# PaddlePaddle/Paddle3D

Measured on AMD Instinct MI355X. Metric: scenes/sec CenterPoint-Pillars nuScenes 300k-pt sweeps, higher is better.
Workload: dtype f32

## Files before the change

include/paddle3d_amd.h:

```cpp
#ifndef PADDLE3D_AMD_H
#define PADDLE3D_AMD_H

#include <stddef.h>
#include <stdint.h>

#ifdef __cplusplus
extern "C" {
#endif

#define PD3_OK 0
#define PD3_EINVAL (-1)
#define PD3_EWORKSPACE (-2)
#define PD3_EUNSUPPORTED (-3)

int pd3_version(void);
const char *pd3_target_arch(void);

int pd3_selfcheck_lds_atomic_order(const uint32_t *addr, uint32_t *old, int blocks, int waves_per_block, int rounds,
                                   int table, void *stream);

size_t pd3_hard_voxelize_workspace(int batch, int64_t max_points, int num_point_dim,
                                   const float *voxel_size, const float *point_cloud_range,
                                   int max_num_points_in_voxel, int max_voxels);
int pd3_hard_voxelize(const float *points, const int32_t *num_points, int batch, int64_t max_points,
                      int num_point_dim, const float *voxel_size, const float *point_cloud_range,
                      int max_num_points_in_voxel, int max_voxels, float *voxels, int32_t *coords,
                      int32_t *num_points_per_voxel, int32_t *num_voxels, int32_t *coors_batched,
                      void *workspace, size_t workspace_bytes, void *stream);
int pd3_hard_voxelize_path(const float *points, const int32_t *num_points, int batch, int64_t max_points,
                           int num_point_dim, const float *voxel_size, const float *point_cloud_range,
                           int max_num_points_in_voxel, int max_voxels, float *voxels, int32_t *coords,
                           int32_t *num_points_per_voxel, int32_t *num_voxels, int32_t *coors_batched,
                           void *workspace, size_t workspace_bytes, void *stream, int path);

int64_t pd3_hard_voxelize_index_list_entries(int batch, int64_t max_points);
int pd3_hard_voxelize_index(const float *points, const int32_t *num_points, int batch, int64_t max_points,
                            int num_point_dim, const float *voxel_size, const float *point_cloud_range,
                            int max_num_points_in_voxel, int max_voxels, int32_t *vox_span, int32_t *point_list,
                            int32_t *coords, int32_t *num_points_per_voxel, int32_t *num_voxels,
                            int32_t *coors_batched, void *workspace, size_t workspace_bytes, void *stream);

int pd3_hard_voxelize_f64(const double *points, const int32_t *num_points, int batch, int64_t max_points,
                          int num_point_dim, const float *voxel_size, const float *point_cloud_range,
                          int max_num_points_in_voxel, int max_voxels, double *voxels, int32_t *coords,
                          int32_t *num_points_per_voxel, int32_t *num_voxels, int32_t *coors_batched,
                          void *workspace, size_t workspace_bytes, void *stream);

int pd3_dynamic_voxelize(const float *points, int64_t num_points, int num_point_dim, const float *voxel_size,
                         const float *point_cloud_range, int32_t *coors, void *stream);

size_t pd3_pointpillars_scatter_workspace(int batch, int ny, int nx);
int pd3_pointpillars_scatter(const float *voxel_features, const int32_t *coords,
                             int64_t num_pillars, int channels, int batch, int ny, int nx,
                             float *canvas, void *workspace, size_t workspace_bytes, void *stream);

int pd3_pointpillars_inverse_map(const int32_t *coords, int64_t num_pillars, int batch, int ny, int nx,
                                 int32_t *inv, void *stream);
int pd3_scatter_conv3x3_bias_relu(const float *voxel_features, const int32_t *inv, const float *w_packed,
                                  const float *bias, int batch, int cin, int cout, int ny, int nx, int stride,
                                  int relu, float *out, int out_w, void *stream);

size_t pd3_pillar_conv_rulebook_workspace(int batch, int ny, int nx, int stride);
int pd3_pillar_conv_rulebook(const int32_t *inverse_map, int batch, int ny, int nx, int stride, int32_t *nbr,
                             int32_t *out_cell, int32_t *cell_row, int32_t *n_out, int capacity, int32_t *order,
                             void *workspace, size_t workspace_bytes, void *stream);
int pd3_rows_to_dense_fill(const float *rows, const int32_t *cell_row, const float *fill, int batch, int channels, int h,
                           int w, float *out, void *stream);

int pd3_pillar_feature_net(const float *voxels, const int32_t *num_points, const int32_t *coors,
                           int64_t num_pillars, int max_points, int num_point_dim,
                           int voxel_center_dims, float vx, float vy, float vz, float x_offset,
                           float y_offset, float z_offset, const float *w1, const float *scale1,
                           const float *shift1, int c1, const float *w2, const float *scale2,
                           const float *shift2, int c2, float *out, void *stream);

int pd3_pillar_feature_net_path(const float *voxels, const int32_t *num_points, const int32_t *coors,
                                int64_t num_pillars, int max_points, int num_point_dim,
                                int voxel_center_dims, float vx, float vy, float vz, float x_offset,
                                float y_offset, float z_offset, const float *w1, const float *scale1,
                                const float *shift1, int c1, const float *w2, const float *scale2,
                                const float *shift2, int c2, float *out, int path, void *stream);

int pd3_pillar_feature_net_indexed(const float *points, int64_t points_per_frame, const int32_t *vox_span,
                                   const int32_t *point_list, int64_t list_stride, const int32_t *coors,
                                   int64_t num_pillars, int pillars_per_frame, int max_points, int num_point_dim,
                                   int voxel_center_dims, float vx, float vy, float vz, float x_offset,
                                   float y_offset, float z_offset, const float *w1, const float *scale1,
                                   const float *shift1, int c1, const float *w2, const float *scale2,
                                   const float *shift2, int c2, float *out, void *stream);

int pd3_voxel_mean(const float *voxels, const int32_t *num_points, int64_t num_voxels,
                   int max_points, int num_point_dim, float *out, void *stream);

size_t pd3_nms_workspace(int num_boxes);
int pd3_nms_bev(const float *boxes, int num_boxes, float nms_overlap_thresh, int32_t *keep,
                int32_t *num_to_keep, void *workspace, size_t workspace_bytes, void *stream);
int pd3_nms_normal(const float *boxes, int num_boxes, float nms_overlap_thresh, int32_t *keep,
                   int32_t *num_to_keep, void *workspace, size_t workspace_bytes, void *stream);
int pd3_boxes_iou_bev(const float *boxes_a, int num_a, const float *boxes_b, int num_b,
                      float *ans_iou, void *stream);
int pd3_boxes_overlap_bev(const float *boxes_a, int num_a, const float *boxes_b, int num_b,
                          float *ans_overlap, void *stream);
int pd3_libm_eval(int op, const float *x, const float *y, float *out, int64_t n, void *stream);

size_t pd3_centerpoint_postprocess_workspace(int batch, int num_tasks, int feat_h, int feat_w,
                                             int nms_pre_max_size, int nms_post_max_size);
int pd3_centerpoint_postprocess(const float *const *hm, const float *const *reg,
                                const float *const *height, const float *const *dim,
                                const float *const *vel, const float *const *rot, int batch,
                                int num_tasks, const int *hm_channels, int feat_h, int feat_w,
                                const float *voxel_size, const float *point_cloud_range,
                                const float *post_center_range, const int *label_offsets,
                                int down_ratio, float score_threshold, float nms_iou_threshold,
                                int nms_pre_max_size, int nms_post_max_size, int with_velocity,
                                float *out_bboxes, float *out_scores, int64_t *out_labels,
                                int32_t *out_count, void *workspace, size_t workspace_bytes,
                                void *stream);

int pd3_centerpoint_postprocess_strided(const float *const *hm, const float *const *reg,
                                const float *const *height, const float *const *dim,
                                const float *const *vel, const float *const *rot, int64_t head_batch_stride, int batch,
                                int num_tasks, const int *hm_channels, int feat_h, int feat_w,
                                const float *voxel_size, const float *point_cloud_range,
                                const float *post_center_range, const int *label_offsets,
                                int down_ratio, float score_threshold, float nms_iou_threshold,
                                int nms_pre_max_size, int nms_post_max_size, int with_velocity,
                                float *out_bboxes, float *out_scores, int64_t *out_labels,
                                int32_t *out_count, void *workspace, size_t workspace_bytes,
                                void *stream, int selection);
int pd3_centerpoint_postprocess_records(const float *const *hm, const float *const *reg,
                                        const float *const *height, const float *const *dim,
                                        const float *const *vel, const float *const *rot,
                                        int64_t head_batch_stride, int batch, int num_tasks,
                                        const int *hm_channels, int feat_h, int feat_w, const float *voxel_size,
                                        const float *point_cloud_range, const float *post_center_range,
                                        const int *label_offsets, int down_ratio, float score_threshold,
                                        float nms_iou_threshold, int nms_pre_max_size, int nms_post_max_size,
                                        int with_velocity, float *out_bboxes, float *out_scores,
                                        int64_t *out_labels, int32_t *out_count, float *out_records,
                                        int max_per_img, void *workspace, size_t workspace_bytes, void *stream);

size_t pd3_bevdet_postprocess_workspace(int batch, int num_tasks, const int *task_classes, int feat_h, int feat_w,
                                        int max_num);
int pd3_bevdet_postprocess(const float *const *heatmap, const float *const *reg, const float *const *height,
                           const float *const *dim, const float *const *rot, const float *const *vel, int batch,
                           int num_tasks, const int *task_classes, int feat_h, int feat_w, const int *nms_type,
                           const float *nms_thr, const double *min_radius, const float *rescale_factors,
                           int max_num, int pre_max_size, int post_max_size, float score_threshold, int norm_bbox,
                           const float *post_center_range, const float *post_center_limit_range,
                           const float *pc_range, const float *voxel_size, float out_size_factor,
// ... 325 lines not shown
```

paddle3d_amd/_lib.py:

```python
from __future__ import annotations

import ctypes as C
import os
from functools import lru_cache

_HERE = os.path.dirname(os.path.abspath(__file__))
LIB_PATH = os.path.join(_HERE, "lib", "libpaddle3d_amd.so")

c_f32p = C.c_void_p
c_i32p = C.c_void_p

_SIGNATURES = {
    "pd3_version": (C.c_int, []),
    "pd3_target_arch": (C.c_char_p, []),
    "pd3_hard_voxelize_workspace": (C.c_size_t, [C.c_int, C.c_int64, C.c_int, C.c_void_p, C.c_void_p,
                                                 C.c_int, C.c_int]),
    "pd3_hard_voxelize": (C.c_int, [C.c_void_p, C.c_void_p, C.c_int, C.c_int64, C.c_int, C.c_void_p,
                                    C.c_void_p, C.c_int, C.c_int, C.c_void_p, C.c_void_p, C.c_void_p,
                                    C.c_void_p, C.c_void_p, C.c_void_p, C.c_size_t, C.c_void_p]),
    "pd3_hard_voxelize_f64": (C.c_int, [C.c_void_p, C.c_void_p, C.c_int, C.c_int64, C.c_int, C.c_void_p,
                                    C.c_void_p, C.c_int, C.c_int, C.c_void_p, C.c_void_p, C.c_void_p,
                                    C.c_void_p, C.c_void_p, C.c_void_p, C.c_size_t, C.c_void_p]),
    "pd3_hard_voxelize_path": (C.c_int, [C.c_void_p, C.c_void_p, C.c_int, C.c_int64, C.c_int, C.c_void_p,
                                         C.c_void_p, C.c_int, C.c_int, C.c_void_p, C.c_void_p, C.c_void_p,
# ... 199 lines not shown

_SIGNATURES_ROI = {
    "pd3_voxel_pool": (C.c_int, [C.c_void_p] * 8 + [C.c_int] * 7 + [C.c_float] + [C.c_int] * 5 + [C.c_void_p] * 2),
    "pd3_roi_grid_points": (C.c_int, [C.c_void_p, C.c_int64, C.c_int, C.c_int] + [C.c_void_p] * 3 + [C.c_int] +
                            [C.c_void_p] * 3),
    "pd3_rcnn_decode_boxes": (C.c_int, [C.c_void_p, C.c_void_p, C.c_int64, C.c_void_p, C.c_void_p]),
    "pd3_class_agnostic_nms_workspace": (C.c_size_t, [C.c_int, C.c_int64, C.c_int]),
    "pd3_class_agnostic_nms": (C.c_int, [C.c_void_p, C.c_void_p, C.c_int, C.c_int64, C.c_int, C.c_int, C.c_float,
                                         C.c_void_p, C.c_int, C.c_float, C.c_int] + [C.c_void_p] * 5 +
                               [C.c_size_t, C.c_void_p]),
}

SYMBOLS_ROI = tuple(_SIGNATURES_ROI)

_SIGNATURES_HEAD = {
    "pd3_grouped_conv3x3_small_counts_slice": (C.c_int, [C.c_void_p, C.c_void_p, C.c_void_p, C.c_int, C.c_int, C.c_int,
                                                         C.c_int, C.c_void_p, C.c_int, C.c_int, C.c_void_p, C.c_int,
                                                         C.c_int, C.c_void_p]),
}

SYMBOLS_HEAD = tuple(_SIGNATURES_HEAD)

_SIGNATURES_PVRCNN = {
    "pd3_stack_sa_pool": (C.c_int, [C.c_void_p] * 11 + [C.c_int] * 5 + [C.c_float, C.c_int] + [C.c_void_p] * 2),
    "pd3_bev_interpolate": (C.c_int, [C.c_void_p, C.c_void_p, C.c_int64] + [C.c_int] * 4 + [C.c_float] * 5 +
                            [C.c_void_p] * 2),
}

SYMBOLS_PVRCNN = tuple(_SIGNATURES_PVRCNN)

_CADDN_GRID = [C.c_int] * 3 + [C.c_void_p] * 2 + [C.c_int, C.c_double, C.c_double]
_CADDN_IN = [C.c_void_p] * 5 + [C.c_int] * 5 + _CADDN_GRID
_SIGNATURES_CADDN = {
    "pd3_frustum_grid": (C.c_int, [C.c_void_p] * 3 + [C.c_int] + _CADDN_GRID + [C.c_int] + [C.c_void_p] * 2),
    "pd3_frustum_to_voxel_workspace": (C.c_size_t, [C.c_int] * 5),
    "pd3_frustum_to_voxel": (C.c_int, _CADDN_IN + [C.c_void_p, C.c_void_p, C.c_size_t, C.c_void_p]),
    "pd3_frustum_to_bev_workspace": (C.c_size_t, [C.c_int] * 7),
    "pd3_frustum_to_bev": (C.c_int, _CADDN_IN + [C.c_void_p] * 3 + [C.c_int, C.c_void_p, C.c_void_p, C.c_size_t,
                                                                    C.c_void_p]),
}

SYMBOLS_CADDN = tuple(_SIGNATURES_CADDN)

_SIGNATURES_BEVFORMER = {
    "pd3_bevformer_point_sampling": (C.c_int, [C.c_void_p] * 3 + [C.c_int] * 6 + [C.c_void_p] * 5),
    "pd3_bevformer_sca": (C.c_int, [C.c_void_p] * 7 + [C.c_int] * 9 + [C.c_void_p] * 2),
    "pd3_bevformer_tsa": (C.c_int, [C.c_void_p] * 6 + [C.c_int] * 7 + [C.c_void_p] * 2),
}

SYMBOLS_BEVFORMER = tuple(_SIGNATURES_BEVFORMER)

_SIGNATURES_BEVFORMER_DEC = {
    "pd3_mha_forward": (C.c_int, [C.c_void_p] * 3 + [C.c_int] * 5 + [C.c_float] + [C.c_void_p] * 2),
    "pd3_bevformer_dec_ca": (C.c_int, [C.c_void_p] * 6 + [C.c_int] * 8 + [C.c_void_p] * 2),
    "pd3_nms_free_decode": (C.c_int, [C.c_void_p] * 3 + [C.c_int] * 5 + [C.c_double, C.c_int] + [C.c_void_p] * 5),
}

SYMBOLS_BEVFORMER_DEC = tuple(_SIGNATURES_BEVFORMER_DEC)

_SIGNATURES_PETR = {
    "pd3_mha_stream_forward": (C.c_int, [C.c_void_p] * 4 + [C.c_int] * 5 + [C.c_float] + [C.c_void_p] * 2),
    "pd3_petr_coords3d": (C.c_int, [C.c_void_p] + [C.c_int] * 6 + [C.c_double, C.c_void_p, C.c_int] + [C.c_void_p] * 4),
}

SYMBOLS_PETR = tuple(_SIGNATURES_PETR)

_SIGNATURES_SQSEG = {
    "pd3_sac_isk_forward": (C.c_int, [C.c_void_p] * 8 + [C.c_int] * 4 + [C.c_void_p] * 2),
    "pd3_range_project": (C.c_int, [C.c_void_p, C.c_int64, C.c_void_p] + [C.c_int] * 3 + [C.c_double] * 2 +
                          [C.c_void_p] * 8 + [C.c_size_t, C.c_void_p]),
}

SYMBOLS_SQSEG = tuple(_SIGNATURES_SQSEG)

_A3D_CFG = [C.c_int] * 2 + [C.c_float] * 4 + [C.c_void_p] * 5 + [C.c_size_t, C.c_void_p]
_SIGNATURES_ANCHOR3D = {
    "pd3_anchor3d_head_workspace": (C.c_size_t, [C.c_int] * 7),
    "pd3_anchor3d_head_forward": (C.c_int, [C.c_void_p] * 8 + [C.c_int] * 7 + _A3D_CFG),
    "pd3_anchor3d_get_bboxes": (C.c_int, [C.c_void_p] * 4 + [C.c_int] * 6 + _A3D_CFG),
}

SYMBOLS_ANCHOR3D = tuple(_SIGNATURES_ANCHOR3D)


class Paddle3DAmdError(RuntimeError):
    pass


@lru_cache(maxsize=None)
def lib() -> C.CDLL:
    if not os.path.exists(LIB_PATH):
        raise Paddle3DAmdError(
            f"{LIB_PATH} not found: build it with `python -m paddle3d_amd.build` "
            "(there is no CPU / PyTorch fallback for the HIP ops)")
    handle = C.CDLL(LIB_PATH)
    for name, (res, args) in (list(_SIGNATURES.items()) + list(_SIGNATURES_ROI.items()) +
                              list(_SIGNATURES_HEAD.items()) + list(_SIGNATURES_PVRCNN.items()) +
                              list(_SIGNATURES_CADDN.items()) + list(_SIGNATURES_BEVFORMER.items()) +
                              list(_SIGNATURES_BEVFORMER_DEC.items()) + list(_SIGNATURES_PETR.items()) +
                              list(_SIGNATURES_SQSEG.items()) + list(_SIGNATURES_ANCHOR3D.items())):
        try:
            fn = getattr(handle, name)
        except AttributeError as e:
            raise Paddle3DAmdError(f"{LIB_PATH} does not export {name}") from e
        fn.restype = res
        fn.argtypes = args
    return handle


def check(status: int, what: str) -> None:
    if status == 0:
        return
    if status < 0:
        msg = {-1: "invalid argument", -2: "workspace too small", -3: "unsupported configuration"}.get(
            status, "error")
        raise Paddle3DAmdError(f"{what}: {msg} (status {status})")
    raise Paddle3DAmdError(f"{what}: HIP error {status}")
```

paddle3d_amd/centerpoint.py:

```python
from __future__ import annotations

import math

import numpy as np
import torch
import torch.nn as nn

from ._lib import Paddle3DAmdError
from .ops import centerpoint_postprocess as _cp
from .ops import conv as _conv
from .ops import pointpillars_scatter as _ps
from .ops import sparse_conv3d as _sp3
from .ops import voxel_encoder as _ve
from .ops import voxelize as _vox

__all__ = ["HardVoxelizer", "PillarFeatureNet", "HardVFE", "VoxelMean", "PointPillarsScatter", "SecondBackbone",
           "SecondFPN", "CenterHead", "CenterPoint", "centerpoint_pillars_nuscenes", "centerpoint_pillars_kitti",
           "centerpoint_voxels_nuscenes", "centerpoint_voxels_kitti", "load_paddle_state_dict"]


def _grid(voxel_size, point_cloud_range):
    pr = np.array(point_cloud_range, dtype=np.float32)
    vs = np.array(voxel_size, dtype=np.float32)
    return np.round((pr[3:] - pr[:3]) / vs).astype(np.int64)
# ... 242 lines not shown
                and _conv.conv3x3_s2_x3_supported(self.cin, self.cout, h, wv, int(x.shape[0]))):
            if "s2x3" not in self.packed:
                self.packed["s2x3"] = _conv.pack_conv3x3_s2_x3_weight(self.w)
            return _conv.conv3x3_s2_x3_bias_relu(x, self.packed["s2x3"], self.b, self.cout, relu=True,
                                                 w_valid=wv), wv // 2
        if _conv.supported(self.cin, self.cout, h, wv, self.stride):
            if "direct" not in self.packed:
                self.packed["direct"] = _conv.pack_conv3x3_weight(self.w)
            return _conv.conv3x3_bias_relu(x, self.packed["direct"], self.b, self.cout, relu=True, stride=self.stride,
                                           w_valid=wv), wv // self.stride
        raise Paddle3DAmdError(f"conv3x3: unsupported configuration (cin {self.cin}, cout {self.cout}, stride "
                               f"{self.stride}, input {h}x{wv}) (status -3)")

    def f16_ok(self, h, w):
        return self.stride == 1 and _conv.f16_supported(self.cin, self.cout, int(h), int(w))

    def f16_s2_ok(self):
        return self.stride == 2 and _conv.s2_f16_supported(self.cin, self.cout)

    def f16_s2(self, x_h):
        if "f16s2" not in self.packed:
            self.packed["f16s2"] = _conv.pack_conv3x3_f16_weight(self.w, tile=128)
        return _conv.conv3x3_s2_f16_bias_relu(x_h, self.packed["f16s2"], self.b, self.cout, relu=True)

    def f16_dual(self, x_h):
        if "f16" not in self.packed:
            self.packed["f16"] = _conv.pack_conv3x3_f16_weight(self.w)
        return _conv.conv3x3_f16_bias_relu_dual(x_h, self.packed["f16"], self.b, self.cout, relu=True)

    def f16(self, x_h, out_f32_nchw=False, out=None, tiles=None, group_major=False):
        if "f16" not in self.packed:
            self.packed["f16"] = _conv.pack_conv3x3_f16_weight(self.w)
        wp, b, cout = self.packed["f16"], self.b, self.cout
        if tiles is not None:
            t = int(wp.shape[4])
            wp, b, cout = wp[tiles[0]:tiles[1]], self.b[tiles[0] * t:tiles[1] * t], (tiles[1] - tiles[0]) * t
        return _conv.conv3x3_f16_bias_relu(x_h, wp, b, cout, relu=True, out_f32_nchw=out_f32_nchw, out=out,
                                           group_major=group_major)


def _valid_w(t) -> int:
    return int(getattr(t, "_pd3_valid_w", t.shape[3]))


def _f16_nhwc_to_f32_nchw(xh):
    x = xh.permute(0, 3, 1, 2).float()
    w = int(x.shape[3])
    pad = _conv.pitch4(w) - w
    if pad:
        x = torch.nn.functional.pad(x, (0, pad))
    return _tag_valid_w(x.contiguous(), w)


def _tag_valid_w(t, wv):
    if t.dtype == torch.float16:
        return t
    if wv != t.shape[3]:
        t._pd3_valid_w = int(wv)
    return t


def _fold_conv3x3(conv, bn):
    if (isinstance(conv, nn.ConvTranspose2d) or tuple(conv.kernel_size) != (3, 3) or tuple(conv.padding) != (1, 1)
            or tuple(conv.stride) not in ((1, 1), (2, 2))):
        raise Paddle3DAmdError(f"unsupported configuration: {conv} is not a 3x3 / pad 1 / stride 1|2 convolution")
    w, b = _fold_conv_bn(conv, bn)
    return _Conv3x3(w, b, conv.stride[0])


class SecondBackbone(_InferenceCache, nn.Module):

    def __init__(self, in_channels=128, out_channels=(128, 128, 256), layer_nums=(3, 5, 5),
                 downsample_strides=(2, 2, 2)):
        super().__init__()
        in_filters = [in_channels, *out_channels[:-1]]
        blocks = []
        for i, n in enumerate(layer_nums):
            block = _conv_bn_relu(in_filters[i], out_channels[i], 3, stride=downsample_strides[i], padding=1)
            for _ in range(n):
                block += _conv_bn_relu(out_channels[i], out_channels[i], 3, padding=1)
            blocks.append(nn.Sequential(*block))
        self.blocks = nn.ModuleList(blocks)
        self.sparse_first = True
        self.amp = False
        self.amp_out_f16 = False

    def _plan(self):
        if not self._cache_valid():
            plan = []
            for blk in self.blocks:
                mods = list(blk)
                plan.append([_fold_conv3x3(mods[i], mods[i + 1]) for i in range(0, len(mods), 3)])
            self._store_cache(plan)
        return self._cache

    def forward(self, x):
        self._require_eval()
        plan = self._plan()
        first = None
        first_h = None
        if isinstance(x, _ps.SparseCanvas):
            c0 = plan[0][0]
            if (self.amp and c0.stride == 2 and x.shape[1] == c0.cin and len(plan[0]) > 1
                    and _conv.scatter_conv_s2_f16_supported(c0.cin, c0.cout, x.ny, x.nx)
                    and plan[0][1].f16_ok(x.ny // 2, x.nx // 2)):
                key = "f16s2_64" if c0.cout % 128 else "f16s2"
                if key not in c0.packed:
                    c0.packed[key] = _conv.pack_conv3x3_f16_weight(c0.w, tile=64 if c0.cout % 128 else 128)
                first_h = _conv.scatter_conv3x3_s2_f16_bias_relu(x, c0.packed[key], c0.b, c0.cout)
                first = (None, x.nx // 2)
            elif (self.sparse_first and x.shape[1] == c0.cin
                  and _conv.scatter_conv_sparse_supported(c0.cin, c0.cout, x.ny, x.nx, c0.stride)):
                y, c0.packed["x3sparse"] = _conv.scatter_conv3x3_sparse(x, c0.w, c0.b, c0.packed.get("x3sparse"))
                first = (y, x.nx // 2)
            elif _conv.scatter_conv_supported(c0.cin, c0.cout, x.ny, x.nx, c0.stride) and x.shape[1] == c0.cin:
                if "direct" not in c0.packed:
                    c0.packed["direct"] = _conv.pack_conv3x3_weight(c0.w)
                first = (_conv.scatter_conv3x3_bias_relu(x, c0.packed["direct"], c0.b, c0.cout), x.nx // 2)
            else:
                x = x.dense()
        if first is None and x.shape[3] % 4:
            raise Paddle3DAmdError(f"SecondBackbone: unsupported configuration (input width {x.shape[3]} is not a "
                                   "multiple of 4) (status -3)")
        outs, wv = [], (0 if first is not None else int(x.shape[3]))
        carry = None
        for bi, layers in enumerate(plan):
            li = 0
            while li < len(layers):
                conv = layers[li]
                xh = None
                if first is not None and bi == 0 and li == 0:
                    x, wv = first
                    li += 1
                    if first_h is None:
                        continue
                    xh = first_h
                    conv = layers[li]
                if self.amp and li == 0 and carry is not None and conv.f16_s2_ok() and wv == carry.shape[2]:
                    xh = conv.f16_s2(carry)
                    li, wv = 1, wv // 2
                    x = None
                carry = None
                if xh is None and x.dtype == torch.float16:
                    x = _f16_nhwc_to_f32_nchw(x)
                h_now = int(xh.shape[1]) if xh is not None else int(x.shape[2])
                w_now = int(xh.shape[2]) if xh is not None else int(x.shape[3])
                run = li
                while (self.amp and run < len(layers) and wv == w_now and layers[run].f16_ok(h_now, w_now)):
                    run += 1
                if run > li and w_now % 4 and not (run == len(layers) and self.amp_out_f16):
                    run = li
                if run > li:
                    if xh is None:
                        xh = _conv.to_f16_nhwc(x)
                    nxt = plan[bi + 1][0] if bi + 1 < len(plan) else None
                    opens = run == len(layers) and nxt is not None and nxt.f16_s2_ok()
                    stage_h = run == len(layers) and self.amp_out_f16
                    for k in range(li, run):
                        if k == run - 1 and stage_h:
                            xh = layers[k].f16(xh)
                            x, carry = xh, (xh if opens else None)
                        elif k == run - 1 and opens:
                            carry, x = layers[k].f16_dual(xh)
                        else:
                            xh = layers[k].f16(xh, out_f32_nchw=(k == run - 1))
                            x = xh
                    li = run
                    continue
                if xh is not None:
                    x = _f16_nhwc_to_f32_nchw(xh)
                    continue
                x, wv = conv(x, wv)
                li += 1
            outs.append(_tag_valid_w(x, wv))
        return tuple(outs)


class SecondFPN(_InferenceCache, nn.Module):

    def __init__(self, in_channels=(128, 128, 256), out_channels=(256, 256, 256), upsample_strides=(1, 2, 4),
                 use_conv_for_no_stride=False):
        super().__init__()
        deblocks = []
        for i, oc in enumerate(out_channels):
            stride = upsample_strides[i]
            if stride > 1 or (stride == 1 and not use_conv_for_no_stride):
                layer = _conv_bn_relu(in_channels[i], oc, int(stride), stride=int(stride), transpose=True)
            else:
                s = round(1 / stride)
                layer = _conv_bn_relu(in_channels[i], oc, s, stride=s)
            deblocks.append(nn.Sequential(*layer))
        self.deblocks = nn.ModuleList(deblocks)

# ... 442 lines not shown
```

paddle3d_amd/ops/conv.py:

```python
from __future__ import annotations

import ctypes

import torch

from ._common import check, lib, ptr, require_gpu, stream_ptr

__all__ = ["pack_conv3x3_weight", "conv3x3_bias_relu", "supported", "pitch4", "pack_grouped_weight", "grouped_conv3x3_small",
           "grouped_small_supported", "winograd_supported", "pack_winograd_weight", "conv3x3_winograd_bias_relu",
           "patch_mode", "patch_supported", "pack_patch_weight", "patch_conv_bias_relu",
           "patch_x3_supported", "pack_patch_weight_x3", "patch_conv_x3_bias_relu", "split_bf16x3",
           "conv3x3_s2_x3_supported", "pack_conv3x3_s2_x3_weight", "conv3x3_s2_x3_bias_relu",
           "winograd43_input_transform", "conv3x3_winograd43_ppv_bias_relu",
           "winograd43_supported", "winograd43_tile", "pack_winograd43_weight", "conv3x3_winograd43_bias_relu",
           "WINOGRAD43_PP_MIN_CIN", "winograd43_pp_supported", "pack_winograd43_lane_weight", "conv3x3_winograd43_pp_bias_relu",
           "f16_supported", "f16_tile", "pack_conv3x3_f16_weight", "conv3x3_f16_bias_relu", "to_f16_nhwc",
           "pack_grouped_weight_f16", "grouped_conv3x3_small_f16", "conv3x3_f16_bias_relu_dual",
           "s2_f16_supported", "conv3x3_s2_f16_bias_relu", "scatter_conv_s2_f16_supported",
           "scatter_conv3x3_s2_f16_bias_relu", "scatter_conv_sparse_supported", "scatter_conv3x3_sparse"]


def pitch4(w: int) -> int:
    return (int(w) + 3) // 4 * 4


def supported(cin: int, cout: int, h: int, w: int, stride: int = 1) -> bool:
    return stride in (1, 2) and cin % 8 == 0 and cout % 64 == 0 and h % stride == 0 and w % stride == 0


def pack_conv3x3_weight(weight: torch.Tensor) -> torch.Tensor:
    cout, cin = weight.shape[:2]
    assert weight.shape[2:] == (3, 3) and cout % 64 == 0 and cin % 8 == 0
    w = weight.reshape(cout // 64, 64, cin // 8, 4, 2, 9).permute(0, 2, 3, 5, 4, 1)
    return w.reshape(cout // 64, cin // 8, 72, 64).contiguous()


def conv3x3_bias_relu(x: torch.Tensor, w_packed: torch.Tensor, bias, cout: int, relu: bool = True,
                      stride: int = 1, out: torch.Tensor | None = None, w_valid: int | None = None) -> torch.Tensor:
    xx = require_gpu(x, "conv3x3_bias_relu")
    n, cin, h, w = xx.shape
    wv = w if w_valid is None else int(w_valid)
    if out is None:
        out = torch.empty((n, cout, h // stride, pitch4(wv // stride)), dtype=torch.float32, device=xx.device)
    check(lib().pd3_conv3x3_bias_relu(ptr(xx), ptr(w_packed), ptr(bias), n, cin, cout, h, w, wv, int(stride),
                                      int(bool(relu)), ptr(out), int(out.shape[3]), stream_ptr(xx.device)),
          "conv3x3_bias_relu")
    return out


def scatter_conv_supported(cin: int, cout: int, ny: int, nx: int, stride: int) -> bool:
    return stride == 2 and cin % 8 == 0 and cout % 64 == 0 and ny % 2 == 0 and nx % 2 == 0


def scatter_conv3x3_bias_relu(canvas, w_packed: torch.Tensor, bias, cout: int, relu: bool = True) -> torch.Tensor:
    f, inv = canvas.features, canvas.inv
    n, cin, ny, nx = canvas.shape
    wo = pitch4(nx // 2)
    out = torch.empty((n, cout, ny // 2, wo), dtype=torch.float32, device=f.device)
    check(lib().pd3_scatter_conv3x3_bias_relu(ptr(f), ptr(inv), ptr(w_packed), ptr(bias), n, cin, cout, ny, nx, 2,
                                              int(bool(relu)), ptr(out), wo, stream_ptr(f.device)),
          "scatter_conv3x3_bias_relu")
    return out


def scatter_conv_sparse_supported(cin: int, cout: int, ny: int, nx: int, stride: int) -> bool:
    ho, wo = (ny - 1) // stride + 1, (nx - 1) // stride + 1
    return stride == 2 and cin % 16 == 0 and cout in (64, 128) and wo % 4 == 0 and (ho * wo) % 4 == 0


def scatter_conv3x3_sparse(canvas, weight: torch.Tensor, bias: torch.Tensor, packed=None, relu: bool = True):
    from . import sparse_conv3d as sp
    from ._common import workspace

    f, inv = canvas.features, canvas.inv
    n, cin, ny, nx = canvas.shape
    cout = int(weight.shape[0])
    ho, wo = (ny - 1) // 2 + 1, (nx - 1) // 2 + 1
    cap = n * ho * wo
    dev = f.device
    L = lib()
    nbr = torch.empty((cap, 9), dtype=torch.int32, device=dev)
    out_cell = torch.empty((cap,), dtype=torch.int32, device=dev)
    cell_row = torch.empty((n, ho * wo), dtype=torch.int32, device=dev)
    n_out = torch.empty((1,), dtype=torch.int32, device=dev)
    ws = workspace(L.pd3_pillar_conv_rulebook_workspace(n, ny, nx, 2), dev)
    order = torch.empty((int(L.pd3_sparse_tile_order_entries(cap)),), dtype=torch.int32, device=dev)
    check(L.pd3_pillar_conv_rulebook(ptr(inv), n, ny, nx, 2, ptr(nbr), ptr(out_cell), ptr(cell_row), ptr(n_out), cap,
                                     ptr(order), ptr(ws), ws.numel(), stream_ptr(dev)), "pillar_conv_rulebook")
    idx = sp.SparseIndices(None, nbr, cap, (1, ho, wo), 9, order, n_out)
    if packed is None:
        packed = sp.pack_weight_bf16x3(weight.permute(2, 3, 1, 0).reshape(1, 3, 3, cin, cout).contiguous())
    rows = sp.features_bf16x3(f, idx, packed, cin, cout, bias, None, None, None, relu)
    fill = torch.relu(bias) if relu else bias
    out = torch.empty((n, cout, ho, wo), dtype=torch.float32, device=dev)
    check(L.pd3_rows_to_dense_fill(ptr(rows), ptr(cell_row), ptr(fill.contiguous()), n, cout, ho, wo, ptr(out),
                                   stream_ptr(dev)), "rows_to_dense_fill")
    return out, packed


def winograd_supported(cin: int, cout: int, h: int, w: int) -> bool:
    return cin % 8 == 0 and cout % 32 == 0 and w % 4 == 0


def pack_winograd_weight(weight: torch.Tensor) -> torch.Tensor:
    cout, cin = weight.shape[:2]
    assert weight.shape[2:] == (3, 3) and cout % 32 == 0 and cin % 8 == 0
    g = torch.tensor([[1.0, 0.0, 0.0], [0.5, 0.5, 0.5], [0.5, -0.5, 0.5], [0.0, 0.0, 1.0]], dtype=torch.float64,
                     device=weight.device)
    u = torch.einsum("ij,ocjk,lk->ocil", g, weight.double(), g).float()
    u = u.reshape(cout // 32, 2, 16, cin // 8, 8, 16).permute(0, 3, 1, 4, 2, 5)
    return u.contiguous()


def conv3x3_winograd_bias_relu(x: torch.Tensor, u_packed: torch.Tensor, bias, cout: int, relu: bool = True,
                               out: torch.Tensor | None = None) -> torch.Tensor:
    xx = require_gpu(x, "conv3x3_winograd_bias_relu")
    n, cin, h, w = xx.shape
    if out is None:
        out = torch.empty((n, cout, h, w), dtype=torch.float32, device=xx.device)
    check(lib().pd3_conv3x3_winograd_bias_relu(ptr(xx), ptr(u_packed), ptr(bias), n, cin, cout, h, w,
                                               int(bool(relu)), ptr(out), stream_ptr(xx.device)),
          "conv3x3_winograd_bias_relu")
    return out


def winograd43_supported(cin: int, cout: int, h: int, w: int) -> bool:
    return cin % 4 == 0 and cout % 32 == 0


def winograd43_tile(cout: int) -> int:
    return 64 if cout % 64 == 0 else 32


def _winograd43_u(weight: torch.Tensor) -> torch.Tensor:
    g = torch.tensor([[1 / 4, 0, 0], [-1 / 6, -1 / 6, -1 / 6], [-1 / 6, 1 / 6, -1 / 6], [1 / 24, 1 / 12, 1 / 6],
                      [1 / 24, -1 / 12, 1 / 6], [0, 0, 1]], dtype=torch.float64, device=weight.device)
    return torch.einsum("ij,ocjk,lk->ocil", g, weight.double(), g).float()


def pack_winograd43_weight(weight: torch.Tensor, tile: int | None = None) -> torch.Tensor:
    cout, cin = weight.shape[:2]
    t = winograd43_tile(cout) if tile is None else tile
    assert weight.shape[2:] == (3, 3) and cout % t == 0 and cin % 4 == 0 and t in (32, 64)
    u = _winograd43_u(weight).reshape(cout // t, t // 16, 16, cin // 4, 4, 36).permute(0, 3, 1, 4, 2, 5)
    return u.contiguous()


def conv3x3_winograd43_bias_relu(x: torch.Tensor, u_packed: torch.Tensor, bias, cout: int, relu: bool = True,
                                 out: torch.Tensor | None = None, w_valid: int | None = None) -> torch.Tensor:
    xx = require_gpu(x, "conv3x3_winograd43_bias_relu")
    n, cin, h, w = xx.shape
    tile = 16 * u_packed.shape[2]
    if out is None:
        out = torch.empty((n, cout, h, w), dtype=torch.float32, device=xx.device)
    check(lib().pd3_conv3x3_winograd43_bias_relu(ptr(xx), ptr(u_packed), ptr(bias), n, cin, cout, h, w,
                                                 w if w_valid is None else int(w_valid), int(bool(relu)), ptr(out),
                                                 tile, stream_ptr(xx.device)),
          "conv3x3_winograd43_bias_relu")
    return out


def patch_mode(weight: torch.Tensor, stride: int, transpose: bool):
    k = weight.shape[2]
    if weight.shape[2] != weight.shape[3] or k != stride:
        return None
    if k == 1:
        return 1
    if k == 2:
        return 2 if transpose else 0
    if k == 4 and transpose:
        return 3
    return None


def patch_supported(mode: int, cin: int, cout: int, h: int, w: int) -> bool:
    if mode == 0:
        return h % 4 == 0 and w % 4 == 0 and (cin * 4) % 16 == 0 and cout % 64 == 0
    if (h * w) % 4 or cin % 16:
        return False
    return {1: cout >= 1, 2: (cout * 4) % 64 == 0, 3: (cout * 16) % 64 == 0}.get(mode, False)


# ... 332 lines not shown
```

Baseline: 2341.

## Add fused span-tiled sparse first conv for pillar backbone

Adds a HIP kernel that computes the stride-2 first backbone conv straight from pillar features and the inverse map. It processes 256-output-cell spans per workgroup, builds per-tap compacted neighbor lists in LDS, and accumulates with bf16x3-split MFMA, then writes bias, ReLU and fill directly into the dense output. This replaces the separate rulebook, sparse-feature and rows-to-dense passes, removing their intermediate buffers and extra launches. It only covers cin 64, cout 64/128 with output width a multiple of 256, and brings added complexity in LDS-heavy scheduling.

```diff
diff --git a/include/paddle3d_amd.h b/include/paddle3d_amd.h
--- a/include/paddle3d_amd.h
+++ b/include/paddle3d_amd.h
@@ -66,6 +66,10 @@
                              void *workspace, size_t workspace_bytes, void *stream);
 int pd3_rows_to_dense_fill(const float *rows, const int32_t *cell_row, const float *fill, int batch, int channels, int h,
                            int w, float *out, void *stream);
+
+int pd3_pillar_conv_span_x3(const float *feats, int n_in, const int32_t *inverse_map, int batch, int ny, int nx, int stride,
+                            int cin, int cout, const void *weight_packed, const float *bias, const float *fill, int relu,
+                            float *out, void *stream);
 
 int pd3_pillar_feature_net(const float *voxels, const int32_t *num_points, const int32_t *coors,
                            int64_t num_pillars, int max_points, int num_point_dim,
diff --git a/paddle3d_amd/_lib.py b/paddle3d_amd/_lib.py
--- a/paddle3d_amd/_lib.py
+++ b/paddle3d_amd/_lib.py
@@ -305,6 +305,13 @@
 
 SYMBOLS_ANCHOR3D = tuple(_SIGNATURES_ANCHOR3D)
 
+_SIGNATURES_SPAN = {
+    "pd3_pillar_conv_span_x3": (C.c_int, [C.c_void_p, C.c_int, C.c_void_p] + [C.c_int] * 6 + [C.c_void_p] * 3 +
+                                [C.c_int] + [C.c_void_p] * 2),
+}
+
+SYMBOLS_SPAN = tuple(_SIGNATURES_SPAN)
+
 
 class Paddle3DAmdError(RuntimeError):
     pass
@@ -321,7 +328,8 @@
                               list(_SIGNATURES_HEAD.items()) + list(_SIGNATURES_PVRCNN.items()) +
                               list(_SIGNATURES_CADDN.items()) + list(_SIGNATURES_BEVFORMER.items()) +
                               list(_SIGNATURES_BEVFORMER_DEC.items()) + list(_SIGNATURES_PETR.items()) +
-                              list(_SIGNATURES_SQSEG.items()) + list(_SIGNATURES_ANCHOR3D.items())):
+                              list(_SIGNATURES_SQSEG.items()) + list(_SIGNATURES_ANCHOR3D.items()) +
+                              list(_SIGNATURES_SPAN.items())):
         try:
             fn = getattr(handle, name)
         except AttributeError as e:
diff --git a/paddle3d_amd/centerpoint.py b/paddle3d_amd/centerpoint.py
--- a/paddle3d_amd/centerpoint.py
+++ b/paddle3d_amd/centerpoint.py
@@ -348,6 +348,8 @@
             blocks.append(nn.Sequential(*block))
         self.blocks = nn.ModuleList(blocks)
         self.sparse_first = True
+        self.sparse_first = True
+        self.span_first = True
         self.amp = False
         self.amp_out_f16 = False
 
@@ -375,6 +377,10 @@
                     c0.packed[key] = _conv.pack_conv3x3_f16_weight(c0.w, tile=64 if c0.cout % 128 else 128)
                 first_h = _conv.scatter_conv3x3_s2_f16_bias_relu(x, c0.packed[key], c0.b, c0.cout)
                 first = (None, x.nx // 2)
+            elif (self.sparse_first and self.span_first and x.shape[1] == c0.cin
+                  and _conv.scatter_conv_span_supported(c0.cin, c0.cout, x.ny, x.nx, c0.stride)):
+                y, c0.packed["x3span"] = _conv.scatter_conv3x3_span(x, c0.w, c0.b, c0.packed.get("x3span"))
+                first = (y, x.nx // 2)
             elif (self.sparse_first and x.shape[1] == c0.cin
                   and _conv.scatter_conv_sparse_supported(c0.cin, c0.cout, x.ny, x.nx, c0.stride)):
                 y, c0.packed["x3sparse"] = _conv.scatter_conv3x3_sparse(x, c0.w, c0.b, c0.packed.get("x3sparse"))
diff --git a/paddle3d_amd/csrc/pillar_conv_span.hip b/paddle3d_amd/csrc/pillar_conv_span.hip
--- /dev/null
+++ b/paddle3d_amd/csrc/pillar_conv_span.hip
@@ -0,0 +1,264 @@
+#include "../../include/paddle3d_amd.h"
+#include "common.hpp"
+
+namespace pd3 {
+
+typedef __bf16 ps_b8 __attribute__((ext_vector_type(8)));
+typedef float ps_f32x16 __attribute__((ext_vector_type(16)));
+typedef float ps_f32x4 __attribute__((ext_vector_type(4)));
+
+constexpr int kPsCells = 256;
+constexpr int kPsPitch = kPsCells + 4;
+constexpr int kPsCh = 64;
+constexpr int kPsCin = 64, kPsKC = 32;
+constexpr int kPsGrid = 512;
+constexpr size_t kPsLds = (size_t)kPsCh * kPsPitch * 4 + 9 * kPsCells * 4 + 9 * kPsCells + 64 * 4 + 4 * 8 + 2 * kPsCh * 4;
+static_assert(2 * kPsLds <= 160 * 1024, "two workgroups per CU");
+
+struct PcSpanArgs {
+  const float* feats;
+  const int32_t* inv;
+  const __bf16* wpk;
+  const float *bias, *fill;
+  float* out;
+  int n_in, batch, ny, nx, ho, wo, cout, relu;
+  int spans;
+};
+
+struct PsRows {
+  ps_f32x4 v[2][2][2];
+  int cell;
+  bool live;
+};
+
+typedef float ps_f32x2 __attribute__((ext_vector_type(2)));
+typedef __bf16 ps_b2 __attribute__((ext_vector_type(2)));
+
+__device__ __forceinline__ void ps_split(ps_f32x4 lo4, ps_f32x4 hi4, bool live, ps_b8& h, ps_b8& m, ps_b8& l) {
+#pragma unroll
+  for (int e = 0; e < 8; e += 2) {
+    const ps_f32x2 x = e < 4 ? ps_f32x2{lo4[e & 3], lo4[(e & 3) + 1]} : ps_f32x2{hi4[e & 3], hi4[(e & 3) + 1]};
+    const ps_b2 a = __builtin_convertvector(x, ps_b2);
+    const ps_f32x2 r1 = x - __builtin_convertvector(a, ps_f32x2);
+    const ps_b2 b = __builtin_convertvector(r1, ps_b2);
+    const ps_f32x2 r2 = r1 - __builtin_convertvector(b, ps_f32x2);
+    const ps_b2 c = __builtin_convertvector(r2, ps_b2);
+    h[e] = a[0], h[e + 1] = a[1];
+    m[e] = b[0], m[e + 1] = b[1];
+    l[e] = c[0], l[e + 1] = c[1];
+  }
+  typedef unsigned ps_u32x4 __attribute__((ext_vector_type(4)));
+  const unsigned keep = live ? ~0u : 0u;
+  h = __builtin_bit_cast(ps_b8, __builtin_bit_cast(ps_u32x4, h) & keep);
+  m = __builtin_bit_cast(ps_b8, __builtin_bit_cast(ps_u32x4, m) & keep);
+  l = __builtin_bit_cast(ps_b8, __builtin_bit_cast(ps_u32x4, l) & keep);
+}
+
+__global__ __launch_bounds__(kPsCells, 2) void pc_span_x3_kernel(PcSpanArgs a) {
+  extern __shared__ __attribute__((aligned(16))) unsigned char ps_smem[];
+  float* tile = reinterpret_cast<float*>(ps_smem);
+  int* nb = reinterpret_cast<int*>(tile + kPsCh * kPsPitch);
+  uint8_t* list = reinterpret_cast<uint8_t*>(nb + 9 * kPsCells);
+  int* cnt = reinterpret_cast<int*>(list + 9 * kPsCells);
+  unsigned long long* act = reinterpret_cast<unsigned long long*>(cnt + 64);
+  float* sbias = reinterpret_cast<float*>(act + 4);
+  float* sfill = sbias + kPsCh;
+  const int t = threadIdx.x, lane = lane_id(), wave = wave_id();
+  const int l31 = lane & 31, kh = lane >> 5;
+  const int uwave = __builtin_amdgcn_readfirstlane(wave) ^ (((int)blockIdx.x / (kPsGrid / 2)) & 1) * 2;
+  const int nh = a.cout / kPsCh, half = blockIdx.x % nh;
+  const int sp_stride = gridDim.x / nh;
+  const int spr = a.wo / kPsCells;
+  const int64_t plane = (int64_t)a.ho * a.wo;
+  const float* fsrc = a.n_in > 0 ? a.feats : reinterpret_cast<const float*>(a.wpk);
+
+  for (int i = t; i < kPsCh * kPsPitch; i += kPsCells) tile[i] = 0.f;
+  if (t < kPsCh) {
+    sbias[t] = a.bias ? a.bias[half * kPsCh + t] : 0.f;
+    sfill[t] = a.fill[half * kPsCh + t];
+  }
+
+  auto load_inv = [&](int sp, int (&j)[9], int& valid) {
+    const int xs = sp % spr, r = sp / spr;
+    const int oy = r % a.ho, b = r / a.ho;
+    const int ix0 = 2 * (xs * kPsCells + t) - 1, iy0 = 2 * oy - 1;
+    valid = 0;
+#pragma unroll
+    for (int k = 0; k < 9; ++k) {
+      const int iy = iy0 + k / 3, ix = ix0 + k % 3;
+      const bool ok = iy >= 0 && iy < a.ny && ix >= 0 && ix < a.nx;
+      valid |= ok ? 1 << k : 0;
+      const int cy = min(max(iy, 0), a.ny - 1), cx = min(max(ix, 0), a.nx - 1);
+      j[k] = a.inv[((int64_t)b * a.ny + cy) * a.nx + cx];
+    }
+  };
+
+  ps_b8 wa[2][2][3];
+  auto load_w = [&](int k) {
+    const ps_b8* w8 = reinterpret_cast<const ps_b8*>(a.wpk) + (half * kPsCh + (uwave & 1) * 32 + l31) * (kPsKC / 8) + kh;
+#pragma unroll
+    for (int c = 0; c < 2; ++c)
+#pragma unroll
+      for (int p = 0; p < 3; ++p)
+#pragma unroll
+        for (int sx = 0; sx < 2; ++sx) wa[c][sx][p] = w8[(int64_t)(k * 6 + c * 3 + p) * a.cout * (kPsKC / 8) + sx * 2];
+  };
+  auto units_of = [&](int k) { return 2 * ((__builtin_amdgcn_readfirstlane(cnt[36 + k]) + 31) >> 5); };
+  auto gather = [&](int k, int blk, PsRows& g) {
+    const int idx = blk * 32 + l31;
+    g.live = idx < cnt[36 + k];
+    g.cell = g.live ? (int)list[k * kPsCells + idx] : 0;
+    const int j = g.live ? nb[k * kPsCells + g.cell] : 0;
+    const ps_f32x4* src = reinterpret_cast<const ps_f32x4*>(fsrc + (int64_t)j * kPsCin + kh * (kPsKC / 2));
+#pragma unroll
+    for (int c = 0; c < 2; ++c)
+#pragma unroll
+      for (int s = 0; s < 2; ++s) {
+        g.v[c][s][0] = src[c * (kPsKC / 4) + 2 * s];
+        g.v[c][s][1] = src[c * (kPsKC / 4) + 2 * s + 1];
+      }
+  };
+  auto unit = [&](const PsRows& g) {
+    float* tl = tile + ((uwave & 1) * 32 + 4 * kh) * kPsPitch + g.cell;
+    ps_f32x16 acc;
+#pragma unroll
+    for (int r = 0; r < 16; ++r) {
+      const float v = tl[((r & 3) + 8 * (r >> 2)) * kPsPitch];
+      acc[r] = g.live ? v : 0.f;
+    }
+#pragma unroll
+    for (int c = 0; c < 2; ++c)
+#pragma unroll
+      for (int s = 0; s < 2; ++s) {
+        ps_b8 b0, b1, b2;
+        const ps_b8(&av)[3] = wa[c][s];
+        ps_split(g.v[c][s][0], g.v[c][s][1], g.live, b0, b1, b2);
+        acc = __builtin_amdgcn_mfma_f32_32x32x16_bf16(av[0], b2, acc, 0, 0, 0);
+        acc = __builtin_amdgcn_mfma_f32_32x32x16_bf16(av[2], b0, acc, 0, 0, 0);
+        acc = __builtin_amdgcn_mfma_f32_32x32x16_bf16(av[1], b1, acc, 0, 0, 0);
+        acc = __builtin_amdgcn_mfma_f32_32x32x16_bf16(av[0], b1, acc, 0, 0, 0);
+        acc = __builtin_amdgcn_mfma_f32_32x32x16_bf16(av[1], b0, acc, 0, 0, 0);
+        acc = __builtin_amdgcn_mfma_f32_32x32x16_bf16(av[0], b0, acc, 0, 0, 0);
+      }
+    if (g.live) {
+#pragma unroll
+      for (int r = 0; r < 16; ++r) tl[((r & 3) + 8 * (r >> 2)) * kPsPitch] = acc[r];
+    }
+  };
+
+  auto step = [&](int k, PsRows& cur, PsRows& nxt) {
+    const int units = units_of(k);
+    const bool then = k < 8 && uwave < units_of(k < 8 ? k + 1 : k);
+    if (k < 8) gather(k + 1, uwave >> 1, nxt);
+    if (uwave < units) unit(cur);
+#pragma clang loop unroll(disable)
+    for (int u = uwave + 4; u < units; u += 4) {
+      gather(k, u >> 1, cur);
+      unit(cur);
+    }
+    if (then) load_w(k + 1);
+    px_lds_barrier();
+  };
+
+  const int g = blockIdx.x / nh, trips = (a.spans + sp_stride - 1) / sp_stride;
+  const int rot = max(sp_stride / trips, 1);
+  auto span_of = [&](int i) {
+    const int sp = i * sp_stride + (g + i * rot) % sp_stride;
+    return i < trips && sp < a.spans ? sp : -1;
+  };
+
+  for (int trip = 0; trip < trips; ++trip) {
+    const int sp = span_of(trip);
+    if (sp < 0) continue;
+    int jn[9], vn;
+    load_inv(sp, jn, vn);
+    __syncthreads();
+    int pos[9], mask = 0;
+#pragma unroll
+    for (int k = 0; k < 9; ++k) {
+      const int j = jn[k];
+      const bool has = ((vn >> k) & 1) && j >= 0 && j < a.n_in;
+      nb[k * kPsCells + t] = has ? j : -1;
+      mask |= has ? 1 << k : 0;
+      const unsigned long long bal = __ballot(has);
+      pos[k] = __popcll(bal & ((1ull << lane) - 1ull));
+      if (lane == 0) cnt[k * 4 + wave] = __popcll(bal);
+    }
+    {
+      const unsigned long long bal = __ballot(mask != 0);
+      if (lane == 0) act[wave] = bal;
+    }
+    __syncthreads();
+#pragma unroll
+    for (int k = 0; k < 9; ++k) {
+      int base = 0;
+#pragma unroll
+      for (int w = 0; w < 3; ++w) base += w < wave ? cnt[k * 4 + w] : 0;
+      if ((mask >> k) & 1) list[k * kPsCells + base + pos[k]] = (uint8_t)t;
+    }
+    if (t < 9) cnt[36 + t] = cnt[t * 4] + cnt[t * 4 + 1] + cnt[t * 4 + 2] + cnt[t * 4 + 3];
+    const bool any = (act[0] | act[1] | act[2] | act[3]) != 0ull;
+    const int xs = sp % spr, r = sp / spr;
+    const int oy = r % a.ho, b = r / a.ho;
+    __syncthreads();
+    if (any) {
+      PsRows ra, rb;
+      gather(0, uwave >> 1, ra);
+      if (uwave < units_of(0)) load_w(0);
+#pragma unroll 1
+      for (int k = 0; k < 8; k += 2) {
+        step(k, ra, rb);
+        step(k + 1, rb, ra);
+      }
+      step(8, ra, rb);
+    }
+    float* o = a.out + ((int64_t)b * a.cout + half * kPsCh) * plane + (int64_t)oy * a.wo + xs * kPsCells;
+#pragma unroll 4
+    for (int it = 0; it < kPsCh * kPsCells / 4 / kPsCells; ++it) {
+      const int e = it * kPsCells + t;
+      const int c = e >> 6, p4 = e & 63;
+      float* tl = tile + c * kPsPitch + p4 * 4;
+      const ps_f32x4 v = *reinterpret_cast<const ps_f32x4*>(tl);
+      const unsigned bits = (unsigned)(act[p4 >> 4] >> ((p4 & 15) * 4)) & 15u;
+      const float bs = sbias[c], fl = sfill[c];
+      ps_f32x4 ov;
+#pragma unroll
+      for (int q = 0; q < 4; ++q) {
+        float x = v[q];
+        if (a.bias) x += bs;
+        if (a.relu) x = fmaxf(x, 0.f);
+        ov[q] = (bits >> q) & 1u ? x : fl;
+      }
+      *reinterpret_cast<ps_f32x4*>(o + c * plane + p4 * 4) = ov;
+      if (any) *reinterpret_cast<ps_f32x4*>(tl) = ps_f32x4{0.f, 0.f, 0.f, 0.f};
+    }
+  }
+}
+
+}
+
+using namespace pd3;
+
+extern "C" int pd3_pillar_conv_span_x3(const float* feats, int n_in, const int32_t* inverse_map, int batch, int ny, int nx,
+                                       int stride, int cin, int cout, const void* weight_packed, const float* bias,
+                                       const float* fill, int relu, float* out, void* stream) {
+  if (!inverse_map || !weight_packed || !fill || !out || n_in < 0 || (n_in > 0 && !feats) || batch <= 0 || ny <= 0 ||
+      nx <= 0 || cin <= 0 || cout <= 0)
+    return PD3_EINVAL;
+  if (stride != 2 || cin != kPsCin || (cout != 64 && cout != 128)) return PD3_EUNSUPPORTED;
+  const int ho = (ny - 1) / 2 + 1, wo = (nx - 1) / 2 + 1;
+  if (wo % kPsCells != 0) return PD3_EUNSUPPORTED;
+  const int64_t spans = (int64_t)batch * ho * (wo / kPsCells);
+  if (spans >= ((int64_t)1 << 30)) return PD3_EUNSUPPORTED;
+  if (reinterpret_cast<uintptr_t>(feats) % 16 != 0 || reinterpret_cast<uintptr_t>(weight_packed) % 16 != 0 ||
+      reinterpret_cast<uintptr_t>(out) % 16 != 0)
+    return PD3_EINVAL;
+  PcSpanArgs a{feats, inverse_map, static_cast<const __bf16*>(weight_packed), bias, fill, out, n_in, batch, ny, nx, ho, wo,
+               cout, relu ? 1 : 0, (int)spans};
+  const int nh = cout / kPsCh;
+  const unsigned grid = (unsigned)(spans < kPsGrid / nh ? spans : kPsGrid / nh) * nh;
+  hipError_t e = pd3_max_dynamic_lds(reinterpret_cast<const void*>(pc_span_x3_kernel), (int)kPsLds);
+  if (e != hipSuccess) return (int)e;
+  pc_span_x3_kernel<<<grid, kPsCells, kPsLds, static_cast<hipStream_t>(stream)>>>(a);
+  return launch_status();
+}
diff --git a/paddle3d_amd/ops/conv.py b/paddle3d_amd/ops/conv.py
--- a/paddle3d_amd/ops/conv.py
+++ b/paddle3d_amd/ops/conv.py
@@ -17,7 +17,8 @@
            "f16_supported", "f16_tile", "pack_conv3x3_f16_weight", "conv3x3_f16_bias_relu", "to_f16_nhwc",
            "pack_grouped_weight_f16", "grouped_conv3x3_small_f16", "conv3x3_f16_bias_relu_dual",
            "s2_f16_supported", "conv3x3_s2_f16_bias_relu", "scatter_conv_s2_f16_supported",
-           "scatter_conv3x3_s2_f16_bias_relu", "scatter_conv_sparse_supported", "scatter_conv3x3_sparse"]
+           "scatter_conv3x3_s2_f16_bias_relu", "scatter_conv_sparse_supported", "scatter_conv3x3_sparse",
+           "scatter_conv_span_supported", "scatter_conv3x3_span"]
 
 
 def pitch4(w: int) -> int:
@@ -98,6 +99,27 @@
     return out, packed
 
 
+def scatter_conv_span_supported(cin: int, cout: int, ny: int, nx: int, stride: int) -> bool:
+    return stride == 2 and cin == 64 and cout in (64, 128) and ((nx - 1) // 2 + 1) % 256 == 0 and ny > 0
+
+
+def scatter_conv3x3_span(canvas, weight: torch.Tensor, bias: torch.Tensor, packed=None, relu: bool = True):
+    from . import sparse_conv3d as sp
+
+    f, inv = canvas.features, canvas.inv
+    n, cin, ny, nx = canvas.shape
+    cout = int(weight.shape[0])
+    if packed is None:
+        packed = (sp.pack_weight_bf16x3(weight.permute(2, 3, 1, 0).reshape(1, 3, 3, cin, cout).contiguous()),
+                  (torch.relu(bias) if relu else bias.clone()).contiguous())
+    wpk, fill = packed
+    out = torch.empty((n, cout, (ny - 1) // 2 + 1, (nx - 1) // 2 + 1), dtype=torch.float32, device=f.device)
+    check(lib().pd3_pillar_conv_span_x3(ptr(f), int(f.shape[0]), ptr(inv), n, ny, nx, 2, cin, cout, ptr(wpk), ptr(bias),
+                                        ptr(fill), int(bool(relu)), ptr(out), stream_ptr(f.device)),
+          "pillar_conv_span_x3")
+    return out, packed
+
+
 def winograd_supported(cin: int, cout: int, h: int, w: int) -> bool:
     return cin % 8 == 0 and cout % 32 == 0 and w % 4 == 0
 
```

Result: faster. 2365, median of 6 (+1.0%).
